# zgbkdlm/fbs

Measured on AMD Instinct MI355X. Metric: particle-steps/sec (N x T per Gibbs sweep), higher is better.
Workload: dtype f32; 1 GPU; 2-D Gaussian bridge toy (BASELINE config 2): N=65536 particles, T=500 steps, ts=linspace(0,2), analytic score, gibbs_kernel eb=True ef=False marg_y=False, conditional killing resampling; one step = one Gibbs sweep of a batch of 4 chain(s) (reference driver default nchains=4, vmapped); nparticles=65536, nsteps=500, nchains=4, du=1, dv=1, parallelism=1 GPU(s) x 4 independent chain(s) each, no collective

## Files before the change

### fbs_amd/csrc/fbsmi_lg.hip

```cpp
#include <hip/hip_runtime.h>

#include <array>
#include <cmath>
#include <cstdlib>
#include <map>
#include <mutex>
#include <new>
#include <string>
#include <utility>
#include <vector>

#include "../../include/fbsmi.h"
#include "fbsmi_device.h"
#include "fbsmi_em_path.h"
#include "fbsmi_host.h"

namespace fbsmi {

constexpr int kMaxNbSweep = 1024;
constexpr int kNumProfKernels = 3;

struct LgDev {
    int C;
    int Ctot, c0;
    int plus1;
    int pin;
    int nz;
    int N;
    int nparticles;
    int du, dv, D, T;
    int nb;
    int levels;
    int eb, ef, store;
    float dt;
    float lw_init;
    const float *G, *g, *sd, *lognorm, *F, *sqQ;
    uint32_t* key;
    uint32_t* keys;
    float* x0;
    float* y0;
    int32_t* bs;
    uint32_t* keytab;
    uint32_t* misc;
    float* xi1;
    float* xi2;
    float* path;
    float* us_star;
    float* vs;
    float* u0;
    float* u1;
    float* lw;
    float* lwn;
    float* w;
    float* cdf;
    float* cdfJ;
    float *bmax, *bsumexp, *bsumw, *bsumJ;
    float *hpW, *hpJ;
    const int32_t* hp_map;
    int wide;
    float* lpw;
    int32_t* anc;
    float* xiw;
    float* uw;
    int lh_w, lh_j;
    float2* trW;
    float2* trWtop;
    float* wfirst;
    float* scal;
    int32_t* As;
    float* uss;
    float* lwss;
    float* usT;
    float* x0n;
    float* usn;
    int32_t* bsn;
    uint8_t* acc;
    float** x0s_slot;
    int32_t* counter;
    int flow;
    int systematic;
    float logn;
    float* ell;
};

constexpr int kHeapLevelsW = 11, kHeapSizeW = 1 << kHeapLevelsW;
constexpr int kHeapLevelsJ = 8, kHeapSizeJ = 1 << kHeapLevelsJ;
constexpr int kMidLv = 3, kMidN = 1 << kMidLv;
constexpr int kTreeNodes = 64;

__device__ __forceinline__ LgDev chain_view(LgDev d, int c) {
    const size_t N = d.N, T = d.T, D = d.D, du = d.du, dv = d.dv, nb = d.nb;
// ... 269 lines not shown
    float a[kBridgeChunk], bt[kBridgeChunk], h[kBridgeChunk], z[kBridgeChunk];
#pragma unroll
    for (int j = 0; j < kBridgeChunk / 4; ++j) {
        a[4 * j] = o.A[j].x; a[4 * j + 1] = o.A[j].y; a[4 * j + 2] = o.A[j].z; a[4 * j + 3] = o.A[j].w;
        bt[4 * j] = o.B[j].x * tg; bt[4 * j + 1] = o.B[j].y * tg; bt[4 * j + 2] = o.B[j].z * tg; bt[4 * j + 3] = o.B[j].w * tg;
        h[4 * j] = o.H[j].x; h[4 * j + 1] = o.H[j].y; h[4 * j + 2] = o.H[j].z; h[4 * j + 3] = o.H[j].w;
        z[4 * j] = o.Z[j].x; z[4 * j + 1] = o.Z[j].y; z[4 * j + 2] = o.Z[j].z; z[4 * j + 3] = o.Z[j].w;
    }
#pragma unroll
    for (int j = 0; j < kBridgeChunk; ++j) {
        if (FULL || j < lim) {
            const float drift = a[j] * x + bt[j];
            x = (x + drift * h[j]) + z[j];
        }
    }
    return x;
}

__global__ void __launch_bounds__(128) k_lg_bridge(LgDev dd, BridgeDev b) {
    const LgDev d = chain_view(dd, blockIdx.y);
    const int c = threadIdx.x;
    if (c >= d.dv) return;
    const float4* sn = reinterpret_cast<const float4*>(b.sn + ((size_t)d.dv * blockIdx.y + c) * b.Rp);
    const float4 *tA = reinterpret_cast<const float4*>(b.tA), *tB = reinterpret_cast<const float4*>(b.tB),
                 *tH = reinterpret_cast<const float4*>(b.tH);
    const float tg = d.vs[c];
    float x = d.vs[(size_t)d.T * d.dv + c];
    const int cpi = b.Np / kBridgeChunk, total = d.T * cpi;
    auto fetch = [&](BridgeOps& o, int g) {
#pragma unroll
        for (int j = 0; j < kBridgeChunk / 4; ++j) {
            const int i = g * (kBridgeChunk / 4) + j;
            o.A[j] = tA[i];
            o.B[j] = tB[i];
            o.H[j] = tH[i];
            o.Z[j] = sn[i];
        }
    };
    int k = 0, m = 0;
    auto fold = [&](const BridgeOps& o) {
        const int lim = b.nsub - m * kBridgeChunk;
        x = lim >= kBridgeChunk ? bridge_chunk<true>(o, x, tg, lim) : bridge_chunk<false>(o, x, tg, lim);
        if (++m == cpi) {
            if (k < d.T - 1) d.vs[(size_t)(d.T - 1 - k) * d.dv + c] = x;
            ++k;
            m = 0;
        }
    };
    BridgeOps p, q;
    fetch(p, 0);
    for (int g = 0; g < total; g += 2) {
        fetch(q, g + 1);
        fold(p);
        if (g + 1 >= total) break;
        fetch(p, g + 2);
        fold(q);
    }
}

template <int DMAX>
struct StepTables {
    const float* G;
    const float* g;
    float sd, sd2, lognorm, dt;
    int du, dv, D;
};

template <int DMAX>
__device__ __forceinline__ StepTables<DMAX> step_tables(const LgDev& d, int s) {
    StepTables<DMAX> t;
    t.G = d.G + (size_t)s * d.D * d.D;
    t.g = d.g + (size_t)s * d.D;
    t.sd = d.sd[s];
    t.sd2 = t.sd * t.sd;
    t.lognorm = d.lognorm[s];
    t.dt = d.dt;
    t.du = d.du;
    t.dv = d.dv;
    t.D = d.D;
    return t;
}

template <int DMAX>
__device__ __forceinline__ void load_row(const LgDev& d, const float* up, int p, float (&u)[DMAX]) {
#pragma unroll
    for (int r = 0; r < DMAX; ++r) u[r] = r < d.du ? up[(size_t)r * d.N + p] : 0.0f;
}

template <int DMAX>
__device__ __forceinline__ float drift_row(const StepTables<DMAX>& t, int r, const float (&u)[DMAX],
                                           const float* __restrict__ v_prev) {
    const float* Gr = t.G + (size_t)r * t.D;
    float acc = t.g[r];
#pragma unroll
    for (int c = 0; c < DMAX; ++c)
        if (c < t.du) acc = fbsmi_fmaf(Gr[c], u[c], acc);
#pragma unroll
    for (int c = 0; c < DMAX; ++c)
        if (c < t.dv) acc = fbsmi_fmaf(Gr[t.du + c], v_prev[c], acc);
    return acc;
}

__device__ __forceinline__ float norm_logpdf(float x, float loc, float sd2, float lognorm) {
    const float dlt = x - loc;
    return (lognorm + (dlt * dlt) / sd2) / -2.0f;
}

template <int DMAX>
__device__ __forceinline__ float lg_loglik(const StepTables<DMAX>& t, const float (&u)[DMAX],
                                           const float* __restrict__ v, const float* __restrict__ v_prev) {
    float acc = 0.0f;
#pragma unroll
    for (int r = 0; r < DMAX; ++r) {
        if (r < t.dv) {
            const float dr = drift_row<DMAX>(t, t.du + r, u, v_prev);
            const float cond_m = v_prev[r] + dr * t.dt;
            const float lp = norm_logpdf(v[r], cond_m, t.sd2, t.lognorm);
            acc = r == 0 ? lp : acc + lp;
        }
    }
    return acc;
}

template <int DMAX>
struct GibbsStep {
    uint32_t a0, a1, b0, b1, t0, t1;
    float u3;
    int i_ref, j_ref;
    const float* up;
    float* un;
    float uref[DMAX];
    StepTables<DMAX> t;
    const float *v_prev, *v, *ustar;
};

template <int DMAX>
__device__ __forceinline__ GibbsStep<DMAX> gibbs_step_entry(const LgDev& d, int s) {
    GibbsStep<DMAX> g;
    const uint32_t* kt = d.keytab + 8 * s;
    g.a0 = kt[0]; g.a1 = kt[1]; g.b0 = kt[2]; g.b1 = kt[3]; g.t0 = kt[6]; g.t1 = kt[7];
    g.u3 = __uint_as_float(kt[4]);
    g.i_ref = d.bs[s];
    g.j_ref = d.bs[s + 1];
    g.up = (s & 1) ? d.u1 : d.u0;
    g.un = (s & 1) ? d.u0 : d.u1;
    return g;
}

template <int DMAX>
__device__ __forceinline__ void gibbs_step_entry_rows(const LgDev& d, int s, GibbsStep<DMAX>& g) {
    load_row<DMAX>(d, g.up, g.i_ref, g.uref);
    g.t = step_tables<DMAX>(d, s);
    g.v_prev = d.vs + (size_t)s * d.dv;
    g.v = d.vs + (size_t)(s + 1) * d.dv;
    g.ustar = d.us_star + (size_t)(s + 1) * d.du;
}

__device__ __forceinline__ int roll_shift(int j_ref, int J, int N) {
    const int shift = (j_ref - J) % N;
    return shift < 0 ? shift + N : shift;
}

__device__ __forceinline__ int roll_source(int m, int shift, int N) {
    const int src = m - shift;
    return src < 0 ? src + N : src;
}

template <int DMAX, bool EARLY>
__device__ __forceinline__ void gibbs_slot_gather(const LgDev& d, const GibbsStep<DMAX>& g, int s, int m, int src, bool killed,
                                                  int red, float (&u)[DMAX], const float* ucand = nullptr, bool live = true) {
    const bool pinned = m == g.j_ref;
    const int a = pinned ? g.i_ref : (killed ? red : src);
    if (killed && !pinned) {
#pragma unroll
        for (int r = 0; r < DMAX; ++r)
            if (r < d.du) u[r] = EARLY ? ucand[r] : g.up[(size_t)r * d.N + a];
    }
    if (pinned) {
#pragma unroll
        for (int r = 0; r < DMAX; ++r) u[r] = g.uref[r];
    }
    if (d.As && live) d.As[(size_t)s * d.N + m] = a;
}

template <int DMAX>
__device__ __forceinline__ float gibbs_slot_finish(const LgDev& d, const GibbsStep<DMAX>& g, int s, int m, const float (&u)[DMAX],
                                                   const float (&xi)[DMAX], bool live = true) {
    const bool pinned = m == g.j_ref;
#pragma unroll
    for (int r = 0; r < DMAX; ++r) {
        if (r < d.du) {
            const float dr = drift_row<DMAX>(g.t, r, u, g.v_prev);
            float x = (u[r] + dr * g.t.dt) + g.t.sd * xi[r];
            if (pinned) x = g.ustar[r];
            if (live) {
                g.un[(size_t)r * d.N + m] = x;
                if (d.uss) d.uss[((size_t)(s + 1) * d.N + m) * d.du + r] = x;
            }
        }
    }
    const float l = live ? lg_loglik<DMAX>(g.t, u, g.v, g.v_prev) : -__builtin_inff();
    if (live) d.lw[m] = l;
    return l;
}

template <int DMAX>
__device__ __forceinline__ void pair_noise(const LgDev& d, const GibbsStep<DMAX>& g, int mA, float (&xiA)[DMAX], float (&xiB)[DMAX]) {
#pragma unroll
    for (int r = 0; r < DMAX; ++r) {
        xiA[r] = 0.0f;
        xiB[r] = 0.0f;
        if (r < d.du) {
            uint32_t lo_, hi_;
            random_bits_pair(g.t0, g.t1, (uint64_t)d.N * d.du, (uint64_t)mA * d.du + r, lo_, hi_);
            xiA[r] = normal_from_bits(lo_);
            xiB[r] = normal_from_bits(hi_);
        }
    }
}

__device__ __forceinline__ void pair_sources(int mA, int j_ref, int J, int N, int (&src)[2]) {
    src[0] = roll_source(mA, roll_shift(j_ref, J, N), N);
    src[1] = src[0] < (N >> 1) ? src[0] + (N >> 1) : src[0] - (N >> 1);
}

template <int DMAX>
__device__ __forceinline__ void pair_uniforms(const GibbsStep<DMAX>& g, int N, const int (&src)[2], float (&u1)[2], float (&u2)[2]) {
    const bool a_low = src[0] < (N >> 1);
    const int pbase = a_low ? src[0] : src[1];
    uint32_t k_lo, k_hi, r_lo, r_hi;
    random_bits_pair(g.a0, g.a1, (uint64_t)N, (uint64_t)pbase, k_lo, k_hi);
    random_bits_pair(g.b0, g.b1, (uint64_t)N, (uint64_t)pbase, r_lo, r_hi);
    u1[0] = fbsmi_bits_to_unit(a_low ? k_lo : k_hi);
    u1[1] = fbsmi_bits_to_unit(a_low ? k_hi : k_lo);
    u2[0] = fbsmi_bits_to_unit(a_low ? r_lo : r_hi);
    u2[1] = fbsmi_bits_to_unit(a_low ? r_hi : r_lo);
}

template <int ITEMS, int DMAX>
__global__ void __launch_bounds__(kBlock) k_lg_init(LgDev dd) {
    const LgDev d = chain_view(dd, blockIdx.y);
    __shared__ float xch[2][4];
    const StepTables<DMAX> t = step_tables<DMAX>(d, 0);
    const int b0 = d.bs[0];
    const int base = (blockIdx.x * kBlock + threadIdx.x) * ITEMS;
    float lv[ITEMS];
#pragma unroll
    for (int i = 0; i < ITEMS; ++i) {
        const int p = base + i;
        lv[i] = -__builtin_inff();
        if (p < d.N) {
            float u[DMAX];
#pragma unroll
            for (int r = 0; r < DMAX; ++r) {
                if (r < d.du) {
                    float v = d.us_star[r];
                    if (d.ef && p != b0)
                        v = normal_at(d.misc[2], d.misc[3], (uint64_t)d.N * d.du, (uint64_t)p * d.du + r);
                    u[r] = v;
                    d.u0[(size_t)r * d.N + p] = v;
                    if (d.uss) d.uss[(size_t)p * d.du + r] = v;
                } else {
                    u[r] = 0.0f;
                }
            }
            const float l = d.ef ? lg_loglik<DMAX>(t, u, d.vs, d.vs + d.dv) : d.lw_init;
            d.lw[p] = l;
            lv[i] = l;
        }
    }
    float m, sx;
    block_lse_partial<ITEMS>(lv, xch[0], xch[1], m, sx);
    if (threadIdx.x == 0) {
        d.bmax[blockIdx.x] = m;
        d.bsumexp[blockIdx.x] = sx;
    }
}

typedef float lg_f4u __attribute__((ext_vector_type(4), aligned(4)));

template <int ITEMS>
__device__ __forceinline__ void chunk_load(const float* __restrict__ p, int base, int n, float fill, float (&x)[ITEMS]) {
    if (ITEMS % 4 == 0 && base + ITEMS <= n) {
#pragma unroll
        for (int i = 0; i < ITEMS; i += 4) {
            const lg_f4u q = *reinterpret_cast<const lg_f4u*>(p + base + i);
            x[i] = q.x; x[i + 1] = q.y; x[i + 2] = q.z; x[i + 3] = q.w;
        }
    } else {
#pragma unroll
        for (int i = 0; i < ITEMS; ++i) x[i] = base + i < n ? p[base + i] : fill;
    }
}

template <int ITEMS>
// ... 664 lines not shown
    float ue[DMAX];
    if (kEarlyRow<DMAX>) {
        const int en = lo + 4 < N ? lo + 4 : N - 1;
#pragma unroll
        for (int r = 0; r < DMAX; ++r) {
            ug[r] = r < d.du ? *reinterpret_cast<const float4*>(up + (size_t)r * N + lo) : make_float4(0.f, 0.f, 0.f, 0.f);
            ue[r] = r < d.du ? up[(size_t)r * N + en] : 0.0f;
        }
    }
    const int red = tree_leaves_walk(w4, lo, q, P, E);
    if (kEarlyRow<DMAX>) {
        const int k = red - lo;
#pragma unroll
        for (int r = 0; r < DMAX; ++r) {
            const float lo2 = (k & 1) ? ug[r].y : ug[r].x, hi2 = (k & 1) ? ug[r].w : ug[r].z;
            ucand[r] = k >= 4 ? ue[r] : ((k & 2) ? hi2 : lo2);
        }
    }
    return red;
}

__device__ __forceinline__ int tree_build_shared(const LgDev& d, const TreeEntry& e, TreeLds& L, bool builder, int i_ref, float u3,
                                                 float w_max, float inv_n, float& last) {
    __shared__ int Jsh;
    __shared__ float lastsh;
    if (builder) {
        float lastb, rootW;
        const int J = tree_build(d, e, L, i_ref, u3, w_max, inv_n, lastb, rootW);
        if (threadIdx.x == 0) {
            Jsh = J;
            lastsh = lastb;
        }
    } else {
#pragma unroll
        for (int k = 0; k < kTreeBuildBarriers; ++k) __syncthreads();
    }
    __syncthreads();
    last = lastsh;
    return Jsh;
}

struct WaveTree {
    float x[4];
    float s01, s23;
    TreePath p;
};

__device__ __forceinline__ float wave_tree_upsweep(WaveTree& t) {
    t.s01 = t.x[0] + t.x[1];
    t.s23 = t.x[2] + t.x[3];
    return wave_upsweep(t.s01 + t.s23, t.p);
}

__device__ __forceinline__ float lane_read(float v, int l) {
    return __builtin_bit_cast(float, __builtin_amdgcn_readlane(__builtin_bit_cast(int, v), l));
}
__device__ __forceinline__ int wave_uniform(int v) { return __builtin_amdgcn_readfirstlane(v); }

__device__ __forceinline__ float wave_tree_left_sum(const TreePath p, int lane) {
    float v = p.ls[5];
    v = (lane & 16) ? p.ls[4] : v;
    v = (lane & 8) ? p.ls[3] : v;
    v = (lane & 4) ? p.ls[2] : v;
    v = (lane & 2) ? p.ls[1] : v;
    v = (lane & 1) ? p.ls[0] : v;
    return v;
}

template <int C>
__device__ __forceinline__ float wave_tree_half(const WaveTree& t, int lo) {
    const int ml = (lo + (1 << C)) >> 2;
    if constexpr (C >= 2) return lane_read(t.p.ls[C - 2], ml);
    else if constexpr (C == 1) return lane_read(t.s01, ml);
    else return (lo & 2) ? lane_read(t.x[2], ml) : lane_read(t.x[0], ml);
}
template <int C>
__device__ __forceinline__ float wave_tree_mid(const float (&y)[4], int lo) {
    const int ml = (lo + (1 << C)) >> 2;
    if constexpr (C >= 2) return lane_read(y[0], ml);
    else if constexpr (C == 1) return lane_read(y[2], ml);
    else return (lo & 2) ? lane_read(y[3], ml) : lane_read(y[1], ml);
}

__device__ __forceinline__ float4 tile_values4(const float* p, int nb, int lane) {
    const int t = 4 * lane;
    if (nb >= 4) return t < nb ? *reinterpret_cast<const float4*>(p + t) : make_float4(0.f, 0.f, 0.f, 0.f);
    return make_float4(t < nb ? p[t] : 0.0f, t + 1 < nb ? p[t + 1] : 0.0f, 0.f, 0.f);
}

struct RoleEntry {
    float4 sj, wf;
    float refsib[8];
};

__device__ __forceinline__ float4 role_entry_loads(const LgDev& d, int i_ref, RoleEntry& e) {
    const int tid = threadIdx.x, nb = d.nb;
    float4 wref = make_float4(0.f, 0.f, 0.f, 0.f);
    if (tid < 64) {
        e.sj = tile_values4(d.bsumJ, nb, tid);
        e.wf = tile_values4(d.wfirst, nb, tid);
        wref = *reinterpret_cast<const float4*>(d.w + i_ref / kBlock * kBlock + 4 * tid);
#pragma unroll
        for (int lv = 0; lv < 8; ++lv) e.refsib[lv] = d.scal[4 + lv];
    }
    return wref;
}

__device__ __forceinline__ float wave_tree_w_side(float4 sw, float4 wf, TreeLds& L) {
    const int lane = threadIdx.x & 63;
    WaveTree t;
    t.x[0] = sw.x; t.x[1] = sw.y; t.x[2] = sw.z; t.x[3] = sw.w;
    const float total = wave_tree_upsweep(t);
    const int t0 = 4 * lane;
    if (lane) L.topW[tree_mid_node(t0)] = make_float2(wave_tree_left_sum(t.p, lane), wf.x);
    L.topW[tree_mid_node(t0 + 1)] = make_float2(t.x[0], wf.y);
    L.topW[tree_mid_node(t0 + 2)] = make_float2(t.s01, wf.z);
    L.topW[tree_mid_node(t0 + 3)] = make_float2(t.x[2], wf.w);
    return total;
}

__device__ __forceinline__ int wave_tree_J(const LgDev& d, const RoleEntry& e, const float4 wref, int i_ref, float u3, float w_max,
                                           float inv_n) {
    const int lane = threadIdx.x & 63, nb = d.nb;
    i_ref = wave_uniform(i_ref);
    const int b_ref = i_ref / kBlock, lb = b_ref >> 2;
    WaveTree t;
    t.x[0] = e.sj.x; t.x[1] = e.sj.y; t.x[2] = e.sj.z; t.x[3] = e.sj.w;
    const float wf[4] = {e.wf.x, e.wf.y, e.wf.z, e.wf.w};
    float jq[4];
#pragma unroll
    for (int i = 0; i < 4; ++i) jq[i] = jprob_pow2(wf[i], w_max, inv_n);
    const float total = wave_tree_upsweep(t);
    const float Ji = fmaxf(1.0f - total, 0.0f);
    float jf[4];
#pragma unroll
    for (int i = 0; i < 4; ++i) jf[i] = (4 * lane + i) * kBlock == i_ref ? Ji : (4 * lane + i < nb ? jq[i] : 0.0f);
    const float tile_ref = tree_fold(Ji, e.refsib);
    float bsib[8];
    {
        const int pos = b_ref & 3;
        const float s0 = (pos & 2) ? ((pos & 1) ? t.x[2] : t.x[3]) : ((pos & 1) ? t.x[0] : t.x[1]);
        bsib[0] = lane_read(s0, lb);
        bsib[1] = lane_read((pos & 2) ? t.s01 : t.s23, lb);
        bsib[2] = lane_read(t.p.ls[0], lb); bsib[3] = lane_read(t.p.ls[1], lb); bsib[4] = lane_read(t.p.ls[2], lb);
        bsib[5] = lane_read(t.p.ls[3], lb); bsib[6] = lane_read(t.p.ls[4], lb); bsib[7] = lane_read(t.p.ls[5], lb);
    }
    const float rootJ = tree_fold(tile_ref, bsib);
    const float q = rootJ * (1.0f - u3);
    const int top_levels = 31 - __builtin_clz(nb);
    float P = 0.0f, E = rootJ;
    int lo = 0;
#define FBSMI_JTOP_LEVEL(C)                                                                 \
    if (C < top_levels) {                                                                   \
        const int mid = lo + (1 << C);                                                      \
        float left = wave_tree_half<C>(t, lo);                                              \
        if (b_ref >= lo && b_ref < mid) left = tree_fold(tile_ref, bsib, C);                \
        lo = wave_uniform(tree_walk(make_float2(left, wave_tree_mid<C>(jf, lo)), q, P, E) ? lo : mid); \
    }
    FBSMI_JTOP_LEVEL(7) FBSMI_JTOP_LEVEL(6) FBSMI_JTOP_LEVEL(5) FBSMI_JTOP_LEVEL(4)
    FBSMI_JTOP_LEVEL(3) FBSMI_JTOP_LEVEL(2) FBSMI_JTOP_LEVEL(1) FBSMI_JTOP_LEVEL(0)
#undef FBSMI_JTOP_LEVEL
    const int lo0 = lo * kBlock;
    float w0 = wref.x, w1 = wref.y, w2 = wref.z, w3 = wref.w;
    if (lo != b_ref) {
        const float4 w4 = *reinterpret_cast<const float4*>(d.w + lo0 + 4 * lane);
        w0 = w4.x; w1 = w4.y; w2 = w4.z; w3 = w4.w;
    }
    const int m0 = lo0 + 4 * lane;
    t.x[0] = m0 == i_ref ? Ji : jprob_pow2(w0, w_max, inv_n);
    t.x[1] = m0 + 1 == i_ref ? Ji : jprob_pow2(w1, w_max, inv_n);
    t.x[2] = m0 + 2 == i_ref ? Ji : jprob_pow2(w2, w_max, inv_n);
    t.x[3] = m0 + 3 == i_ref ? Ji : jprob_pow2(w3, w_max, inv_n);
    wave_tree_upsweep(t);
    lo = 0;
#define FBSMI_JTILE_LEVEL(C) \
    lo = wave_uniform(tree_walk(make_float2(wave_tree_half<C>(t, lo), wave_tree_mid<C>(t.x, lo)), q, P, E) ? lo : lo + (1 << C));
    FBSMI_JTILE_LEVEL(7) FBSMI_JTILE_LEVEL(6) FBSMI_JTILE_LEVEL(5) FBSMI_JTILE_LEVEL(4) FBSMI_JTILE_LEVEL(3) FBSMI_JTILE_LEVEL(2)
#undef FBSMI_JTILE_LEVEL
    const int ml = lo >> 2;
    const float x0 = lane_read(t.x[0], ml), x2 = lane_read(t.x[2], ml), s01 = lane_read(t.s01, ml);
    const bool g1 = tree_walk(make_float2(s01, x2), q, P, E);
    const float tt = P + (g1 ? x0 : x2);
    const bool gl = q <= E;
    E = gl ? tt : E;
    const int leaf = lo0 + lo + (g1 ? 0 : 2) + (gl ? 0 : 1);
    return q <= E ? leaf : leaf + 1;
}

__device__ __forceinline__ int tree_build_roles(const LgDev& d, const RoleEntry& e, const float4 wref, TreeLds& L, int i_ref, float u3,
                                                float w_max, float inv_n, float& last) {
    __shared__ int Jsh;
    __shared__ float lastsh;
    const int tid = threadIdx.x, lane = tid & 63, wv = tid >> 6, nb = d.nb;
    if (wv == 0) {
        const int J = wave_tree_J(d, e, wref, i_ref, u3, w_max, inv_n);
        if (lane == 0) Jsh = J;
    } else if (wv == 1) {
        const float total = wave_tree_w_side(tile_values4(d.bsumw, nb, lane), tile_values4(d.wfirst, nb, lane), L);
        if (lane == 0) lastsh = total;
    } else if (wv < 4) {
        constexpr int STN = 2 * 64, STK = kMidN / 2 * kBlock / STN;
        float4 stg[STK];
#pragma unroll
        for (int k = 0; k < STK; ++k) {
            const int idx = tid - 2 * 64 + STN * k;
            stg[k] = idx < kMidN / 2 * nb ? reinterpret_cast<const float4*>(d.trWtop)[idx] : make_float4(0.f, 0.f, 0.f, 0.f);
        }
#pragma unroll
        for (int k = 0; k < STK; ++k) {
            const int idx = tid - 2 * 64 + STN * k;
            if (idx < kMidN / 2 * nb) reinterpret_cast<float4*>(L.midW)[idx] = stg[k];
        }
    }
    __syncthreads();
    last = lastsh;
    return Jsh;
}

template <int DMAX, int HALVES>
__global__ void __launch_bounds__(kBlock * HALVES) k_lg_prop1t(LgDev dd, int s) {
    const LgDev d = chain_view(dd, blockIdx.y);
    __shared__ TreeLds L;
    __shared__ float part[2][4 * HALVES];
    const int N = d.N, tid = threadIdx.x & (kBlock - 1), half = threadIdx.x / kBlock;
    int bx = blockIdx.x;
    if (dd.pin) {
        if (blockIdx.x & 7) return;
        bx = blockIdx.x >> 3;
    }
    const int tileb = bx * HALVES + half;
    const int m = tileb * kBlock + tid;
    const bool live = m < N;
    GibbsStep<DMAX> g = gibbs_step_entry<DMAX>(d, s);
    const float w_max = d.scal[1];
    const float inv_n = 1.0f / (float)N;
    TreeEntry te{};
    if (half == 0) te = tree_entry_loads(d);
    gibbs_step_entry_rows<DMAX>(d, s, g);
    float xi[DMAX];
#pragma unroll
    for (int r = 0; r < DMAX; ++r)
        xi[r] = r < d.du ? normal_at(g.t0, g.t1, (uint64_t)N * d.du, (uint64_t)(live ? m : 0) * d.du + r) : 0.0f;
    float last, rootW;
    int J;
    if (HALVES == 1) {
        J = tree_build(d, te, L, g.i_ref, g.u3, w_max, inv_n, last, rootW);
    } else {
        J = tree_build_shared(d, te, L, half == 0, g.i_ref, g.u3, w_max, inv_n, last);
        rootW = last;
    }
    const int src = live ? roll_source(m, roll_shift(g.j_ref, J, N), N) : 0;
    const float ws = d.w[src];
    float u[DMAX];
    load_row<DMAX>(d, g.up, src, u);
    const float u1 = uniform_at(g.a0, g.a1, (uint64_t)N, (uint64_t)src);
    const float u2 = uniform_at(g.b0, g.b1, (uint64_t)N, (uint64_t)src);
    const float q = last * (1.0f - u2);
    float P = 0.0f, E = rootW;
    int tile, h, red = 0;
    tree_search_lds(L, d.nb - d.plus1, q, P, E, tile, h);
    const bool killed = live && u1 * w_max >= ws;
    float ucand[DMAX];
    if (killed) red = tree_redraw<DMAX>(d, g.up, tile, h, q, P, E, ucand);
    gibbs_slot_gather<DMAX, kEarlyRow<DMAX>>(d, g, s, m, src, killed, red, u, ucand, live);
    const float l = gibbs_slot_finish<DMAX>(d, g, s, m, u, xi, live);
    float mx, sx;
    block_lse_partial_tiles(l, part[0], part[1], mx, sx);
    if (tid == 0) {
        d.bmax[tileb] = mx;
        d.bsumexp[tileb] = sx;
    }
}

template <int DMAX>
constexpr bool kPairNoise = DMAX <= 4;

template <int DMAX, int HALVES>
__global__ void __launch_bounds__(kBlock * HALVES) k_lg_prop1tp(LgDev dd, int s) {
    static_assert(HALVES == 2 || HALVES == 4, "two sides of HALVES / 2 tiles");
    constexpr int HP = HALVES / 2, NP = kBlock * HP;
    const LgDev d = chain_view(dd, blockIdx.y);
// ... 19 lines not shown
            if (r < d.du) xi[r] = normal_at(g.t0, g.t1, (uint64_t)N * d.du, (uint64_t)m * d.du + r);
    } else if (upper) {
#pragma unroll
        for (int r = 0; r < DMAX; ++r) {
            if (r < d.du) {
                uint32_t lo_, hi_;
                random_bits_pair(g.t0, g.t1, (uint64_t)N * d.du, (uint64_t)mL * d.du + r, lo_, hi_);
                xish[r][pr] = normal_from_bits(lo_);
                xi[r] = normal_from_bits(hi_);
            }
        }
    }
    float last;
    const int J = tree_build_shared(d, te, L, half == 0, g.i_ref, g.u3, w_max, inv_n, last);
    const int src = roll_source(m, roll_shift(g.j_ref, J, N), N);
    const float ws = d.w[src];
    float u[DMAX];
    load_row<DMAX>(d, g.up, src, u);
    if (kPairNoise<DMAX> && !upper) {
#pragma unroll
        for (int r = 0; r < DMAX; ++r)
            if (r < d.du) xi[r] = xish[r][pr];
    }
    const float u1 = uniform_at(g.a0, g.a1, (uint64_t)N, (uint64_t)src);
    const float u2 = uniform_at(g.b0, g.b1, (uint64_t)N, (uint64_t)src);
    const float q = last * (1.0f - u2);
    float P = 0.0f, E = last;
    int tile, h, red = 0;
    tree_search_lds(L, d.nb, q, P, E, tile, h);
    const bool killed = u1 * w_max >= ws;
    float ucand[DMAX];
    if (killed) red = tree_redraw<DMAX>(d, g.up, tile, h, q, P, E, ucand);
    gibbs_slot_gather<DMAX, kEarlyRow<DMAX>>(d, g, s, m, src, killed, red, u, ucand);
    const float l = gibbs_slot_finish<DMAX>(d, g, s, m, u, xi);
    float mx, sx;
    block_lse_partial_tiles(l, part[0], part[1], mx, sx);
    if (tid == 0) {
        d.bmax[tileb] = mx;
        d.bsumexp[tileb] = sx;
    }
}

__device__ __forceinline__ float halfwave_max(float m) {
    m = fmaxf(m, tree_partner<1>(m));
    m = fmaxf(m, tree_partner<2>(m));
    m = fmaxf(m, tree_partner<4>(m));
    m = fmaxf(m, tree_partner<8>(m));
    m = fmaxf(m, tree_partner<16>(m));
    return m;
}

__device__ __forceinline__ float halfwave_sum(float s) {
    const int lane = threadIdx.x & 63;
#define FBSMI_HALFWAVE_LEVEL(m, M)                      \
    {                                                   \
        const float o_ = tree_partner<M>(s);            \
        s = ((lane >> m) & 1) ? o_ + s : s + o_;        \
    }
    FBSMI_HALFWAVE_LEVEL(0, 1)
    FBSMI_HALFWAVE_LEVEL(1, 2)
    FBSMI_HALFWAVE_LEVEL(2, 4)
    FBSMI_HALFWAVE_LEVEL(3, 8)
    FBSMI_HALFWAVE_LEVEL(4, 16)
#undef FBSMI_HALFWAVE_LEVEL
    return s;
}

template <int DMAX, int HALVES, bool ROLES>
__global__ void __launch_bounds__(kBlock * HALVES) k_lg_prop1th(LgDev dd, int s) {
    static_assert(HALVES == 2 || HALVES == 4, "two sides of HALVES / 2 tiles");
    constexpr int HP = HALVES / 2, NP = kBlock * HP;
    const LgDev d = chain_view(dd, blockIdx.y);
    __shared__ TreeLds L;
    __shared__ __attribute__((aligned(16))) float part[2][2][HP][8];
    __shared__ float xish[kPairNoise<DMAX> ? DMAX : 1][2 * NP];
    const int N = d.N, hN = N >> 1, tid = threadIdx.x, lane = threadIdx.x & 63, wv = threadIdx.x >> 6;
    const int hw = lane >> 5;
    const bool builder = tid < kBlock;
    const int pr = wv * 32 + (lane & 31);
    const int mL = blockIdx.x * NP + pr;
    const int m = mL + (hw ? hN : 0);
    const int ts = wv >> 3, bk = wv & 7;
    const int tileb = blockIdx.x * HP + ts + (hw ? d.nb >> 1 : 0);
    GibbsStep<DMAX> g = gibbs_step_entry<DMAX>(d, s);
    const float w_max = d.scal[1];
    const float inv_n = 1.0f / (float)N;
    TreeEntry te{};
    RoleEntry re;
    float4 wref = make_float4(0.f, 0.f, 0.f, 0.f);
    if (ROLES) wref = role_entry_loads(d, g.i_ref, re);
    else if (builder) te = tree_entry_loads(d);
    gibbs_step_entry_rows<DMAX>(d, s, g);
    float xi[DMAX] = {};
    if (!kPairNoise<DMAX>) {
#pragma unroll
        for (int r = 0; r < DMAX; ++r)
            if (r < d.du) xi[r] = normal_at(g.t0, g.t1, (uint64_t)N * d.du, (uint64_t)m * d.du + r);
    } else if (tid >= NP) {
        const int p = tid - NP, own = (p >> 5) * 64 + (p & 31);
        const int mp = blockIdx.x * NP + p;
#pragma unroll
        for (int r = 0; r < DMAX; ++r) {
            if (r < d.du) {
                uint32_t lo_, hi_;
                random_bits_pair(g.t0, g.t1, (uint64_t)N * d.du, (uint64_t)mp * d.du + r, lo_, hi_);
                xish[r][own] = normal_from_bits(lo_);
                xish[r][own + 32] = normal_from_bits(hi_);
            }
        }
    }
    float last;
    const int J = ROLES ? tree_build_roles(d, re, wref, L, g.i_ref, g.u3, w_max, inv_n, last)
                        : tree_build_shared(d, te, L, builder, g.i_ref, g.u3, w_max, inv_n, last);
    const int src = roll_source(m, roll_shift(g.j_ref, J, N), N);
    const float ws = d.w[src];
    float u[DMAX];
    load_row<DMAX>(d, g.up, src, u);
    if (kPairNoise<DMAX>) {
#pragma unroll
        for (int r = 0; r < DMAX; ++r)
            if (r < d.du) xi[r] = xish[r][tid];
    }
    const int c = src & (hN - 1);
    const bool swp = (src >= hN) != (hw != 0);
    uint32_t o0, o1;
    threefry2x32(hw ? g.b0 : g.a0, hw ? g.b1 : g.a1, (uint32_t)c, (uint32_t)(c + hN), o0, o1);
    const auto xw = __builtin_amdgcn_permlane32_swap(swp ? o1 : o0, swp ? o0 : o1, false, false);
    const float u1 = fbsmi_bits_to_unit(xw[0]);
    const float u2 = fbsmi_bits_to_unit(xw[1]);
    const float q = last * (1.0f - u2);
    float P = 0.0f, E = last;
    int tile, h, red = 0;
    tree_search_lds(L, d.nb, q, P, E, tile, h);
    const bool killed = u1 * w_max >= ws;
    float ucand[DMAX];
    if (killed) red = tree_redraw<DMAX>(d, g.up, tile, h, q, P, E, ucand);
    gibbs_slot_gather<DMAX, kEarlyRow<DMAX>>(d, g, s, m, src, killed, red, u, ucand);
    const float l = gibbs_slot_finish<DMAX>(d, g, s, m, u, xi);
    float mx, sx;
    {
        const float mw = halfwave_max(l);
        if ((lane & 31) == 0) part[0][hw][ts][bk] = mw;
        __syncthreads();
        const float4 ma = *reinterpret_cast<const float4*>(&part[0][hw][ts][0]);
        const float4 mb = *reinterpret_cast<const float4*>(&part[0][hw][ts][4]);
        mx = fmaxf(fmaxf(fmaxf(ma.x, ma.y), fmaxf(ma.z, ma.w)), fmaxf(fmaxf(mb.x, mb.y), fmaxf(mb.z, mb.w)));
        const float sw_ = halfwave_sum(fbsmi_expf(l - finite_or_zero_f(mx)));
        if ((lane & 31) == 0) part[1][hw][ts][bk] = sw_;
        __syncthreads();
        const float4 sa = *reinterpret_cast<const float4*>(&part[1][hw][ts][0]);
        const float4 sb = *reinterpret_cast<const float4*>(&part[1][hw][ts][4]);
        sx = ((sa.x + sa.y) + (sa.z + sa.w)) + ((sb.x + sb.y) + (sb.z + sb.w));
    }
    if (bk == 0 && (lane & 31) == 0) {
        d.bmax[tileb] = mx;
        d.bsumexp[tileb] = sx;
    }
}

template <int DMAX>
__global__ void __launch_bounds__(kBlock) k_lg_prop2t(LgDev dd, int s) {
    const LgDev d = chain_view(dd, blockIdx.y);
    __shared__ TreeLds L;
    __shared__ float xch2[2][8];
    const int N = d.N, tid = threadIdx.x;
    const int mA = blockIdx.x * kBlock + tid;
    const int m[2] = {mA, mA + (N >> 1)};
    GibbsStep<DMAX> g = gibbs_step_entry<DMAX>(d, s);
    const float w_max = d.scal[1];
    const float inv_n = 1.0f / (float)N;
    const TreeEntry te = tree_entry_loads(d);
    gibbs_step_entry_rows<DMAX>(d, s, g);
    float xi[2][DMAX];
    pair_noise<DMAX>(d, g, mA, xi[0], xi[1]);
    float last;
    float rootW_unused;
    const int J = tree_build(d, te, L, g.i_ref, g.u3, w_max, inv_n, last, rootW_unused);
    int src[2];
    pair_sources(mA, g.j_ref, J, N, src);
    float ws[2], u[2][DMAX];
#pragma unroll
    for (int h2 = 0; h2 < 2; ++h2) {
        ws[h2] = d.w[src[h2]];
#pragma unroll
        for (int r = 0; r < DMAX; ++r) u[h2][r] = r < d.du ? g.up[(size_t)r * N + src[h2]] : 0.0f;
    }
    float u1[2], u2[2];
    pair_uniforms<DMAX>(g, N, src, u1, u2);
    const float qK[2] = {last * (1.0f - u2[0]), last * (1.0f - u2[1])};
    float P[2] = {0.0f, 0.0f}, E[2] = {last, last};
    int tile[2], h[2], hi[2] = {0, 0};
    {
        auto walk2x2 = [&](const float2* hp0, const float2* hp1, int& h0, int& h1) {
            const float2 a0 = hp0[h0], a1 = hp1[h1];
            const float4 c0 = *reinterpret_cast<const float4*>(hp0 + 2 * h0), c1 = *reinterpret_cast<const float4*>(hp1 + 2 * h1);
            const bool g0 = tree_walk(a0, qK[0], P[0], E[0]), g1 = tree_walk(a1, qK[1], P[1], E[1]);
            const bool k0 = tree_walk(g0 ? make_float2(c0.x, c0.y) : make_float2(c0.z, c0.w), qK[0], P[0], E[0]);
            const bool k1 = tree_walk(g1 ? make_float2(c1.x, c1.y) : make_float2(c1.z, c1.w), qK[1], P[1], E[1]);
            h0 = 4 * h0 + (g0 ? 0 : 2) + (k0 ? 0 : 1);
            h1 = 4 * h1 + (g1 ? 0 : 2) + (k1 ? 0 : 1);
        };
        auto walk1x2 = [&](const float2* hp0, const float2* hp1, int& h0, int& h1) {
            const float2 n0 = hp0[h0], n1 = hp1[h1];
            h0 = 2 * h0 + (tree_walk(n0, qK[0], P[0], E[0]) ? 0 : 1);
// ... 2944 lines not shown
```

Baseline: 21.21 billion particle-steps/s.

## Preload per-step tables into uniform registers and split tile loads for DMAX=1

For the one-dimensional case, the per-step drift matrix, offsets, noise scale and observation values are now loaded by value at kernel entry and pinned into scalar registers with readfirstlane and inline-asm constraints, instead of being read through pointers inside the per-particle loops. The du bound becomes a compile-time 1. Role-entry tile loads are split into an early issue of float2 pairs and a later masked unpacking, and the reference-tile load is separated out, so global loads are issued before the tree build and can overlap with it. This trades extra scalar register pressure and more fragile code, with asm hints that constrain the compiler, for fewer dependent loads on the critical path.

```diff
diff --git a/fbs_amd/csrc/fbsmi_lg.hip b/fbs_amd/csrc/fbsmi_lg.hip
--- a/fbs_amd/csrc/fbsmi_lg.hip
+++ b/fbs_amd/csrc/fbsmi_lg.hip
@@ -7,6 +7,7 @@
 #include <mutex>
 #include <new>
 #include <string>
+#include <type_traits>
 #include <utility>
 #include <vector>
 
@@ -442,9 +443,66 @@
 }
 
 template <int DMAX>
+__device__ __forceinline__ int step_du(const LgDev& d) { return DMAX == 1 ? 1 : d.du; }
+
+template <int DMAX>
+constexpr bool kStepByValue = DMAX == 1;
+
+template <int DMAX>
+struct StepValues {
+    float G[2][2];
+    float g[2];
+    float sd, sd2, lognorm, dt;
+};
+
+template <int DMAX>
+struct StepVec {
+    float x[1];
+    __device__ __forceinline__ float operator[](int i) const { return x[i]; }
+};
+
+template <int DMAX>
+__device__ __forceinline__ StepVec<DMAX> step_vec(const float* p) {
+    StepVec<DMAX> v;
+    v.x[0] = p[0];
+    return v;
+}
+
+template <int DMAX>
+__device__ __forceinline__ StepValues<DMAX> step_values(const LgDev& d, int s) {
+    StepValues<DMAX> t;
+    const float* G = d.G + (size_t)s * 4;
+    const float* g = d.g + (size_t)s * 2;
+#pragma unroll
+    for (int r = 0; r < 2; ++r) {
+        t.g[r] = g[r];
+        t.G[r][0] = G[2 * r];
+        t.G[r][1] = G[2 * r + 1];
+    }
+    t.sd = d.sd[s];
+    t.sd2 = t.sd * t.sd;
+    t.lognorm = d.lognorm[s];
+    t.dt = d.dt;
+    return t;
+}
+
+template <class T>
+__device__ __forceinline__ T as_uniform(T v) {
+    if constexpr (sizeof(T) == 4) return __builtin_bit_cast(T, __builtin_amdgcn_readfirstlane(__builtin_bit_cast(int, v)));
+    else return v;
+}
+template <class A, class T>
+__device__ __forceinline__ void pin_uniform(A& anchor, const T& v) {
+    anchor = as_uniform(anchor);
+    asm("" : "+s"(anchor) : "s"(as_uniform(v)));
+}
+template <class A, class... Ts>
+__device__ __forceinline__ void pin_uniforms(A& anchor, const Ts&... vs) { (pin_uniform(anchor, vs), ...); }
+
+template <int DMAX>
 __device__ __forceinline__ void load_row(const LgDev& d, const float* up, int p, float (&u)[DMAX]) {
 #pragma unroll
-    for (int r = 0; r < DMAX; ++r) u[r] = r < d.du ? up[(size_t)r * d.N + p] : 0.0f;
+    for (int r = 0; r < DMAX; ++r) u[r] = r < step_du<DMAX>(d) ? up[(size_t)r * d.N + p] : 0.0f;
 }
 
 template <int DMAX>
@@ -480,6 +538,21 @@
         }
     }
     return acc;
+}
+
+template <int DMAX>
+__device__ __forceinline__ float drift_row(const StepValues<DMAX>& t, int r, const float (&u)[DMAX], const StepVec<DMAX>& v_prev,
+                                           bool vrow = false) {
+    const int R = vrow ? 1 : 0;
+    return fbsmi_fmaf(t.G[R][1], v_prev[0], fbsmi_fmaf(t.G[R][0], u[0], t.g[R]));
+}
+
+template <int DMAX>
+__device__ __forceinline__ float lg_loglik(const StepValues<DMAX>& t, const float (&u)[DMAX], const StepVec<DMAX>& v,
+                                           const StepVec<DMAX>& v_prev) {
+    const float dr = drift_row<DMAX>(t, 0, u, v_prev, true);
+    const float cond_m = v_prev[0] + dr * t.dt;
+    return norm_logpdf(v[0], cond_m, t.sd2, t.lognorm);
 }
 
 template <int DMAX>
@@ -490,8 +563,8 @@
     const float* up;
     float* un;
     float uref[DMAX];
-    StepTables<DMAX> t;
-    const float *v_prev, *v, *ustar;
+    std::conditional_t<kStepByValue<DMAX>, StepValues<DMAX>, StepTables<DMAX>> t;
+    std::conditional_t<kStepByValue<DMAX>, StepVec<DMAX>, const float*> v_prev, v, ustar;
 };
 
 template <int DMAX>
@@ -504,16 +577,27 @@
     g.j_ref = d.bs[s + 1];
     g.up = (s & 1) ? d.u1 : d.u0;
     g.un = (s & 1) ? d.u0 : d.u1;
+    if constexpr (kStepByValue<DMAX>) {
+        g.t = step_values<DMAX>(d, s);
+        g.v_prev = step_vec<DMAX>(d.vs + s);
+        g.v = step_vec<DMAX>(d.vs + s + 1);
+        g.ustar = step_vec<DMAX>(d.us_star + s + 1);
+    }
     return g;
 }
 
 template <int DMAX>
 __device__ __forceinline__ void gibbs_step_entry_rows(const LgDev& d, int s, GibbsStep<DMAX>& g) {
     load_row<DMAX>(d, g.up, g.i_ref, g.uref);
-    g.t = step_tables<DMAX>(d, s);
-    g.v_prev = d.vs + (size_t)s * d.dv;
-    g.v = d.vs + (size_t)(s + 1) * d.dv;
-    g.ustar = d.us_star + (size_t)(s + 1) * d.du;
+    if constexpr (kStepByValue<DMAX>) {
+        pin_uniforms(g.t1, g.t.g[0], g.t.G[0][0], g.t.G[0][1], g.t.g[1], g.t.G[1][0], g.t.G[1][1], g.t.sd, g.t.lognorm,
+                     g.a0, g.a1, g.b0, g.b1, g.t0, g.u3, g.j_ref, g.v_prev.x[0], g.v.x[0], g.ustar.x[0], g.uref[0]);
+    } else {
+        g.t = step_tables<DMAX>(d, s);
+        g.v_prev = d.vs + (size_t)s * d.dv;
+        g.v = d.vs + (size_t)(s + 1) * d.dv;
+        g.ustar = d.us_star + (size_t)(s + 1) * d.du;
+    }
 }
 
 __device__ __forceinline__ int roll_shift(int j_ref, int J, int N) {
@@ -534,7 +618,7 @@
     if (killed && !pinned) {
 #pragma unroll
         for (int r = 0; r < DMAX; ++r)
-            if (r < d.du) u[r] = EARLY ? ucand[r] : g.up[(size_t)r * d.N + a];
+            if (r < step_du<DMAX>(d)) u[r] = EARLY ? ucand[r] : g.up[(size_t)r * d.N + a];
     }
     if (pinned) {
 #pragma unroll
@@ -549,7 +633,7 @@
     const bool pinned = m == g.j_ref;
 #pragma unroll
     for (int r = 0; r < DMAX; ++r) {
-        if (r < d.du) {
+        if (r < step_du<DMAX>(d)) {
             const float dr = drift_row<DMAX>(g.t, r, u, g.v_prev);
             float x = (u[r] + dr * g.t.dt) + g.t.sd * xi[r];
             if (pinned) x = g.ustar[r];
@@ -570,7 +654,7 @@
     for (int r = 0; r < DMAX; ++r) {
         xiA[r] = 0.0f;
         xiB[r] = 0.0f;
-        if (r < d.du) {
+        if (r < step_du<DMAX>(d)) {
             uint32_t lo_, hi_;
             random_bits_pair(g.t0, g.t1, (uint64_t)d.N * d.du, (uint64_t)mA * d.du + r, lo_, hi_);
             xiA[r] = normal_from_bits(lo_);
@@ -1401,28 +1485,42 @@
     else return (lo & 2) ? lane_read(y[3], ml) : lane_read(y[1], ml);
 }
 
-__device__ __forceinline__ float4 tile_values4(const float* p, int nb, int lane) {
+struct TileQuad {
+    float2 lo, hi;
+};
+
+__device__ __forceinline__ TileQuad tile_values4_issue(const float* p, int nb, int lane) {
     const int t = 4 * lane;
-    if (nb >= 4) return t < nb ? *reinterpret_cast<const float4*>(p + t) : make_float4(0.f, 0.f, 0.f, 0.f);
-    return make_float4(t < nb ? p[t] : 0.0f, t + 1 < nb ? p[t + 1] : 0.0f, 0.f, 0.f);
+    TileQuad q;
+    q.lo = *reinterpret_cast<const float2*>(p + (t < nb ? t : nb - 2));
+    q.hi = *reinterpret_cast<const float2*>(p + (t + 2 < nb ? t + 2 : nb - 2));
+    return q;
+}
+
+__device__ __forceinline__ float4 tile_values4(const TileQuad q, int nb, int lane) {
+    const bool a = 4 * lane < nb, b = 4 * lane + 2 < nb;
+    return make_float4(a ? q.lo.x : 0.0f, a ? q.lo.y : 0.0f, b ? q.hi.x : 0.0f, b ? q.hi.y : 0.0f);
 }
 
 struct RoleEntry {
-    float4 sj, wf;
+    TileQuad sj, wf;
     float refsib[8];
+    float w_max;
 };
 
-__device__ __forceinline__ float4 role_entry_loads(const LgDev& d, int i_ref, RoleEntry& e) {
+__device__ __forceinline__ void role_entry_loads(const LgDev& d, RoleEntry& e) {
     const int tid = threadIdx.x, nb = d.nb;
-    float4 wref = make_float4(0.f, 0.f, 0.f, 0.f);
     if (tid < 64) {
-        e.sj = tile_values4(d.bsumJ, nb, tid);
-        e.wf = tile_values4(d.wfirst, nb, tid);
-        wref = *reinterpret_cast<const float4*>(d.w + i_ref / kBlock * kBlock + 4 * tid);
+        e.sj = tile_values4_issue(d.bsumJ, nb, tid);
+        e.wf = tile_values4_issue(d.wfirst, nb, tid);
+        e.w_max = d.scal[1];
 #pragma unroll
         for (int lv = 0; lv < 8; ++lv) e.refsib[lv] = d.scal[4 + lv];
     }
-    return wref;
+}
+
+__device__ __forceinline__ float4 role_entry_ref_tile(const LgDev& d, int i_ref) {
+    return *reinterpret_cast<const float4*>(d.w + i_ref / kBlock * kBlock + 4 * (threadIdx.x & 63));
 }
 
 __device__ __forceinline__ float wave_tree_w_side(float4 sw, float4 wf, TreeLds& L) {
@@ -1444,8 +1542,9 @@
     i_ref = wave_uniform(i_ref);
     const int b_ref = i_ref / kBlock, lb = b_ref >> 2;
     WaveTree t;
-    t.x[0] = e.sj.x; t.x[1] = e.sj.y; t.x[2] = e.sj.z; t.x[3] = e.sj.w;
-    const float wf[4] = {e.wf.x, e.wf.y, e.wf.z, e.wf.w};
+    const float4 sj = tile_values4(e.sj, nb, lane), wf4 = tile_values4(e.wf, nb, lane);
+    t.x[0] = sj.x; t.x[1] = sj.y; t.x[2] = sj.z; t.x[3] = sj.w;
+    const float wf[4] = {wf4.x, wf4.y, wf4.z, wf4.w};
     float jq[4];
 #pragma unroll
     for (int i = 0; i < 4; ++i) jq[i] = jprob_pow2(wf[i], w_max, inv_n);
@@ -1507,15 +1606,16 @@
 }
 
 __device__ __forceinline__ int tree_build_roles(const LgDev& d, const RoleEntry& e, const float4 wref, TreeLds& L, int i_ref, float u3,
-                                                float w_max, float inv_n, float& last) {
+                                                float inv_n, float& last) {
     __shared__ int Jsh;
     __shared__ float lastsh;
     const int tid = threadIdx.x, lane = tid & 63, wv = tid >> 6, nb = d.nb;
     if (wv == 0) {
-        const int J = wave_tree_J(d, e, wref, i_ref, u3, w_max, inv_n);
+        const int J = wave_tree_J(d, e, wref, i_ref, u3, e.w_max, inv_n);
         if (lane == 0) Jsh = J;
     } else if (wv == 1) {
-        const float total = wave_tree_w_side(tile_values4(d.bsumw, nb, lane), tile_values4(d.wfirst, nb, lane), L);
+        const TileQuad sw = tile_values4_issue(d.bsumw, nb, lane), wf = tile_values4_issue(d.wfirst, nb, lane);
+        const float total = wave_tree_w_side(tile_values4(sw, nb, lane), tile_values4(wf, nb, lane), L);
         if (lane == 0) lastsh = total;
     } else if (wv < 4) {
         constexpr int STN = 2 * 64, STK = kMidN / 2 * kBlock / STN;
@@ -1701,26 +1801,27 @@
     const int m = mL + (hw ? hN : 0);
     const int ts = wv >> 3, bk = wv & 7;
     const int tileb = blockIdx.x * HP + ts + (hw ? d.nb >> 1 : 0);
+    TreeEntry te{};
+    RoleEntry re;
     GibbsStep<DMAX> g = gibbs_step_entry<DMAX>(d, s);
     const float w_max = d.scal[1];
+    if (ROLES) role_entry_loads(d, re);
     const float inv_n = 1.0f / (float)N;
-    TreeEntry te{};
-    RoleEntry re;
     float4 wref = make_float4(0.f, 0.f, 0.f, 0.f);
-    if (ROLES) wref = role_entry_loads(d, g.i_ref, re);
+    if (ROLES) wref = role_entry_ref_tile(d, g.i_ref);
     else if (builder) te = tree_entry_loads(d);
     gibbs_step_entry_rows<DMAX>(d, s, g);
     float xi[DMAX] = {};
     if (!kPairNoise<DMAX>) {
 #pragma unroll
         for (int r = 0; r < DMAX; ++r)
-            if (r < d.du) xi[r] = normal_at(g.t0, g.t1, (uint64_t)N * d.du, (uint64_t)m * d.du + r);
+            if (r < step_du<DMAX>(d)) xi[r] = normal_at(g.t0, g.t1, (uint64_t)N * d.du, (uint64_t)m * d.du + r);
     } else if (tid >= NP) {
         const int p = tid - NP, own = (p >> 5) * 64 + (p & 31);
         const int mp = blockIdx.x * NP + p;
 #pragma unroll
         for (int r = 0; r < DMAX; ++r) {
-            if (r < d.du) {
+            if (r < step_du<DMAX>(d)) {
                 uint32_t lo_, hi_;
                 random_bits_pair(g.t0, g.t1, (uint64_t)N * d.du, (uint64_t)mp * d.du + r, lo_, hi_);
                 xish[r][own] = normal_from_bits(lo_);
@@ -1729,7 +1830,7 @@
         }
     }
     float last;
-    const int J = ROLES ? tree_build_roles(d, re, wref, L, g.i_ref, g.u3, w_max, inv_n, last)
+    const int J = ROLES ? tree_build_roles(d, re, wref, L, g.i_ref, g.u3, inv_n, last)
                         : tree_build_shared(d, te, L, builder, g.i_ref, g.u3, w_max, inv_n, last);
     const int src = roll_source(m, roll_shift(g.j_ref, J, N), N);
     const float ws = d.w[src];
@@ -1738,7 +1839,7 @@
     if (kPairNoise<DMAX>) {
 #pragma unroll
         for (int r = 0; r < DMAX; ++r)
-            if (r < d.du) xi[r] = xish[r][tid];
+            if (r < step_du<DMAX>(d)) xi[r] = xish[r][tid];
     }
     const int c = src & (hN - 1);
     const bool swp = (src >= hN) != (hw != 0);
```

Result: faster. 21.85 billion particle-steps/s (median of 6 runs) (+3.0%).
